# zju3dv/neuralbody

Measured on AMD Instinct MI355X. Metric: ray_samples_per_sec, higher is better.
Workload: dtype f16+f6/f4

## Files before the change

### neuralbody_amd/csrc/nb_march_fold.hip

```cpp
#include "nb_f6_ops.h"
#include "nb_march_hooks.h"

using namespace nbm;

namespace {

#ifndef NB_FP4_TERMS
#define NB_FP4_TERMS 3
#endif
constexpr bool FP4_K[2] = {(NB_FP4_TERMS & 1) != 0, (NB_FP4_TERMS & 2) != 0};
constexpr bool ANY_FP4 = FP4_K[0] || FP4_K[1];
constexpr int TERM_ORDER[2] = {(FP4_K[0] && !FP4_K[1]) ? 1 : 0, (FP4_K[0] && !FP4_K[1]) ? 0 : 1};
__host__ __device__ constexpr int term_pieces(int k) { return FP4_K[k] ? 1 : 2; }
__host__ __device__ constexpr int block_pieces(int mt) { return (4 * mt + mt * term_pieces(0) + mt * term_pieces(1) + 1) & ~1; }
__host__ __device__ constexpr int cross_piece(int mt, int slot, int m) {
    return 4 * mt + (slot == 0 ? 0 : mt * term_pieces(TERM_ORDER[0])) + m * term_pieces(TERM_ORDER[slot]);
}
constexpr int S_R = 8;
__host__ __device__ constexpr int phase_pieces(int nb, int mt) { return nb * block_pieces(mt); }
constexpr int N_PH = 4;
constexpr int PH_NB[N_PH] = {4, 4, 4, 2};
constexpr int PH_MT[N_PH] = {2, 2, 1, 1};
__host__ __device__ constexpr int phase_p0(int ph) {
    int p = 0;
// ... 411 lines not shown
            int worst = 0;
#pragma unroll
            for (int w = 0; w < NW; ++w)
                worst = max(worst, __builtin_amdgcn_readlane(n16[w], 0) + __builtin_amdgcn_readlane(n16[w], 16) +
                                       __builtin_amdgcn_readlane(n16[w], 32) + __builtin_amdgcn_readlane(n16[w], 48));
            p.tier = worst <= K_CAP ? 1 : 2;
        }
    }
    return p;
}

struct TblLoad {
    int rid[2], idx[2];
};
__device__ __forceinline__ TblLoad tbl_issue(const Prep &p, const Lvl &lv, int wave, int os) {
    TblLoad t;
    const float rcp_xy = __builtin_amdgcn_rcpf((float)max(p.nxy, 1)), rcp_x = __builtin_amdgcn_rcpf((float)max(p.nx, 1));
#pragma unroll
    for (int q = 0; q < 2; ++q) {
        const int j = 64 * q + 16 * wave + os;
        t.rid[q] = -1;
        t.idx[q] = -1;
        if (j < p.n) {
            const int vz = (int)(((float)j + 0.5f) * rcp_xy);
            const int r = mad24(vz, -p.nxy, j);
            const int vy = (int)(((float)r + 0.5f) * rcp_x);
            const int vx = mad24(vy, -p.nx, r);
            const int lin = mad24(mad24(p.zlo + vz, lv.H, p.ylo + vy), lv.W, p.xlo + vx);
            t.rid[q] = lv.grid[lin];
            t.idx[q] = p.k0 + j;
        }
    }
    return t;
}
__device__ __forceinline__ void tbl_store(char *actz, const TblLoad &t, const Lvl &lv, unsigned zero_off, int K, int tid) {
    unsigned *tbl = reinterpret_cast<unsigned *>(actz + TBL_OFF);
#pragma unroll
    for (int q = 0; q < 2; ++q)
        if (t.idx[q] >= 0) tbl[t.idx[q]] = t.rid[q] < 0 ? zero_off : (unsigned)(lv.rbase + t.rid[q]) << 10;
    if (tid < 16 && K + tid < ((K + 15) & ~15)) tbl[K + tid] = zero_off;
}
__device__ __forceinline__ void tbl_pass(char *actz, unsigned zero_off, int k_lo, int K, int tid) {
    if (tid >= K_CAP) return;
    unsigned *tbl = reinterpret_cast<unsigned *>(actz + TBL_OFF);
    const int k = k_lo + tid;
    unsigned e = zero_off;
    if (k < K) {
        const int k1 = *reinterpret_cast<const int *>(actz + LVL_OFF + 1 * 32 + 20), k2 = *reinterpret_cast<const int *>(actz + LVL_OFF + 2 * 32 + 20),
                  k3 = *reinterpret_cast<const int *>(actz + LVL_OFF + 3 * 32 + 20);
        const int L = (k >= k1) + (k >= k2) + (k >= k3);
        const i32x4 *lp = reinterpret_cast<const i32x4 *>(actz + LVL_OFF + L * 32);
        const i32x4 b0 = lp[0], b1 = lp[1];
        const Lvl lv = load_lvl(actz, L);
        const int j = k - b1.y;
        const float rcp_xy = __builtin_amdgcn_rcpf((float)max(b1.x, 1)), rcp_x = __builtin_amdgcn_rcpf((float)max(b0.w, 1));
        const int vz = (int)(((float)j + 0.5f) * rcp_xy);
        const int r = mad24(vz, -b1.x, j);
        const int vy = (int)(((float)r + 0.5f) * rcp_x);
        const int vx = mad24(vy, -b0.w, r);
        const int lin = mad24(mad24(b0.z + vz, lv.H, b0.y + vy), lv.W, b0.x + vx);
        const int rid = lv.grid[lin];
        if (rid >= 0) e = (unsigned)(lv.rbase + rid) << 10;
    }
    tbl[tid] = e;
}
__device__ __forceinline__ void lvl_store(char *actz, const Prep &p, int tid, int os, int part) {
    if (tid < 64 && os == 0) {
        i32x4 *d = reinterpret_cast<i32x4 *>(actz + LVL_OFF + part * 32);
        d[0] = i32x4{p.xlo, p.ylo, p.zlo, p.nx};
        d[1] = i32x4{p.nxy, p.k0, p.n, 0};
    }
    if (tid == 0) *reinterpret_cast<int *>(actz + HDR_OFF) = p.K;
}

__device__ __forceinline__ unsigned live_chunks(const char *actz, int lane, int nch, unsigned zero_off) {
    typedef unsigned u32x2 __attribute__((ext_vector_type(2)));
    const u32x2 e = reinterpret_cast<const u32x2 *>(actz + TBL_OFF)[lane];
    const unsigned long long b = __builtin_amdgcn_ballot_w64(lane < 8 * nch && (e.x != zero_off || e.y != zero_off));
    auto half = [](unsigned x) -> unsigned {
        x |= x >> 4;
        x |= x >> 2;
        x |= x >> 1;
        return ((x & 0x01010101u) * 0x00204081u >> 21) & 0xfu;
    };
    return half((unsigned)b) | half((unsigned)(b >> 32)) << 4;
}
__device__ __forceinline__ int pop_chunk(unsigned &m) {
    const int c = __builtin_ctz(m);
    m &= m - 1u;
    return c;
}

struct UCfg {
    int nch, R;
    unsigned live;
    int n_live;
    unsigned ring;
    int ring_off;
};
__device__ __forceinline__ UCfg ucfg_k(int K, unsigned live, unsigned lds_base, int wave) {
    UCfg u;
    u.nch = (K + 15) >> 4;
    const int r = u.nch <= 3 ? u.nch : (u.nch == 4 ? 3 : 2);
    u.live = live;
    u.n_live = __builtin_popcount(live);
    u.R = min(r, u.n_live);
    u.ring_off = WT_CHUNK * u.nch + wave * r * U_CHUNK;
    u.ring = lds_base + (unsigned)u.ring_off;
    return u;
}
__device__ __forceinline__ int list_len(const char *actz) {
    return __builtin_amdgcn_readfirstlane(*reinterpret_cast<const int *>(actz + HDR_OFF));
}
__device__ __forceinline__ void dma_chunk(const MarchArgs &a, const char *actz, int lane, int wave, int c, unsigned dst) {
    const int v = ((lane >> 4) << 2) | ((lane >> 1) & 3);
    const unsigned e = *reinterpret_cast<const unsigned *>(actz + TBL_OFF + (16 * c + v) * 4);
    const unsigned voff0 = e + (unsigned)(64 * wave + 16 * ((lane >> 3) & 1) + 8 * (lane & 1)) * 2u;
    const char *base = a.fold.urows;
#pragma unroll
    for (int form = 0; form < 2; ++form)
#pragma unroll
        for (int m = 0; m < 2; ++m) {
            const unsigned voff = voff0 + form * 512 + m * 64;
            const unsigned d = dst + form * 2048 + m * 1024;
            asm volatile(
                "s_mov_b32 m0, %2\n\t"
                "s_nop 0\n\t"
                "global_load_lds_dwordx4 %0, %1"
                :
                : "v"(voff), "s"(base), "s"(d)
                : "memory", "m0");
        }
}
__device__ __forceinline__ void dma_initial(const MarchArgs &a, const char *actz, int lane, int wave, const UCfg &u) {
    unsigned rest = u.live;
    for (int c = 0; c < u.R; ++c) dma_chunk(a, actz, lane, wave, pop_chunk(rest), u.ring + c * U_CHUNK);
}
__device__ __forceinline__ void dma_wait() { asm volatile("s_waitcnt vmcnt(0)" ::: "memory"); }

__device__ __forceinline__ void wt_build(char *actz, const Lvl &lv, const GridCoord &g, bool take, int wave, int os, int part, int nch,
                                         int k_lo = 0) {
    const int nt = wave >> 1, n = 16 * (wave & 1) + os;
    {
        char *z = actz + (part >> 1) * 2048 + nt * 1024 + ((part & 1) * 32 + n) * 16;
        for (int c = 0; c < nch; ++c) *reinterpret_cast<i32x4 *>(z + c * WT_CHUNK) = i32x4{0, 0, 0, 0};
    }
    if (take) {
        const i32x4 *lp = reinterpret_cast<const i32x4 *>(actz + LVL_OFF + part * 32);
        const i32x4 b0 = lp[0], b1 = lp[1];
        const LvlIdx q = level_index(lv, g);
        const float fx = (float)q.x0, fy = (float)q.y0, fz = (float)q.z0;
        const float wx[2] = {(fx + 1.f) - q.ix, q.ix - fx};
        const float wy[2] = {(fy + 1.f) - q.iy, q.iy - fy};
        const float wz[2] = {(fz + 1.f) - q.iz, q.iz - fz};
        const int kbase = b1.y - k_lo + mad24(q.z0 - b0.z, b1.x, mad24(q.y0 - b0.y, b0.w, q.x0 - b0.x));
        const int sbase = nt * 1024 + n * 16;
        float cw[8];
        int ad[8];
#pragma unroll
        for (int corner = 0; corner < 8; ++corner) {
            const int dx = corner & 1, dy = (corner >> 1) & 1, dz = corner >> 2;
            const int xx = q.x0 + dx, yy = q.y0 + dy, zz = q.z0 + dz;
            const bool inb = (unsigned)xx < (unsigned)lv.W && (unsigned)yy < (unsigned)lv.H && (unsigned)zz < (unsigned)lv.D;
            cw[corner] = (wx[dx] * wy[dy]) * wz[dz];
            const int k = kbase + dx + dy * b0.w + dz * b1.x;
            const int off = ((k << 8) & ~0xfff) | ((k << 6) & 0x200) | ((k << 1) & 0xe);
            ad[corner] = (inb && (unsigned)k < (unsigned)(16 * nch)) ? off + sbase : DUMMY_OFF;
        }
#pragma unroll
        for (int cp = 0; cp < 4; ++cp) {
            const unsigned h = cvt_pk_f16(cw[2 * cp], cw[2 * cp + 1]);
            const unsigned l = cvt_pk_f16(rem16<0>(cw[2 * cp], h), rem16<1>(cw[2 * cp + 1], h));
            *reinterpret_cast<unsigned short *>(actz + ad[2 * cp]) = (unsigned short)(h & 0xffffu);
            *reinterpret_cast<unsigned short *>(actz + ad[2 * cp + 1]) = (unsigned short)(h >> 16);
            *reinterpret_cast<unsigned short *>(actz + ad[2 * cp] + 2048) = (unsigned short)(l & 0xffffu);
            *reinterpret_cast<unsigned short *>(actz + ad[2 * cp + 1] + 2048) = (unsigned short)(l >> 16);
        }
    }
}

__device__ __forceinline__ f16x8 tr_frag(const char *p) {
    const s4v a = __builtin_amdgcn_ds_read_tr16_b64_v4i16((lds_s4p)(p));
    const s4v b = __builtin_amdgcn_ds_read_tr16_b64_v4i16((lds_s4p)(p + 256));
    typedef short s8v __attribute__((ext_vector_type(8)));
    return __builtin_bit_cast(f16x8, s8v{a[0], a[1], a[2], a[3], b[0], b[1], b[2], b[3]});
}
struct FoldFrags {
    f16x8 ah[2], al[2];
    i32x4 bh[2], bl[2];
};
__device__ __forceinline__ void fold_wait(int younger) {
    if (younger >= 2) asm volatile("s_waitcnt vmcnt(8)" ::: "memory");
    else if (younger == 1) asm volatile("s_waitcnt vmcnt(4)" ::: "memory");
    else asm volatile("s_waitcnt vmcnt(0)" ::: "memory");
}
__device__ __forceinline__ void fold_read(FoldFrags &f, const char *ub, const char *wtc) {
#pragma unroll
    for (int m = 0; m < 2; ++m) {
        f.ah[m] = tr_frag(ub + m * 1024);
        f.al[m] = tr_frag(ub + 2048 + m * 1024);
    }
#pragma unroll
    for (int n = 0; n < 2; ++n) {
        f.bh[n] = *reinterpret_cast<const i32x4 *>(wtc + n * 1024);
        f.bl[n] = *reinterpret_cast<const i32x4 *>(wtc + 2048 + n * 1024);
    }
}
__device__ __forceinline__ void fold_mma(const FoldFrags &f, f32x16 (&acc)[2][2]) {
#pragma unroll
    for (int p = 0; p < 3; ++p)
#pragma unroll
        for (int m = 0; m < 2; ++m)
#pragma unroll
            for (int n = 0; n < 2; ++n)
                acc[m][n] = __builtin_amdgcn_mfma_f32_32x32x16_f16(p == 2 ? f.al[m] : f.ah[m], __builtin_bit_cast(f16x8, p == 1 ? f.bl[n] : f.bh[n]),
                                                                   acc[m][n], 0, 0, 0);
}
__device__ __forceinline__ void fold_mfma(const MarchArgs &a, char *actz, int lane, int wave, const UCfg &u, f32x16 (&acc)[2][2],
                                          unsigned *tbuf = nullptr) {
    if (u.n_live == 0) return;
    FOLD_SUB(17);
    const int l15 = lane & 15, g4 = lane >> 4;
    const int tro = (g4 >> 1) * 512 + (g4 & 1) * 128 + (l15 >> 2) * 32 + (l15 & 3) * 8;
    const char *wt = actz + lane * 16;
    const char *ring = actz + u.ring_off + tro;
    int issued = u.R - 1;
    unsigned to_read = u.live, to_fetch = u.live;
    for (int c = 0; c < u.R; ++c) to_fetch &= to_fetch - 1u;
    FoldFrags f0, f1;
    fold_wait(issued);
    FOLD_SUB(18);
    fold_read(f0, ring, wt + pop_chunk(to_read) * WT_CHUNK);
    NB_HOOK_FOLD_FIRST_READ(f0);
    FOLD_SUB(19);
    auto step = [&](FoldFrags &cur, FoldFrags &nxt, int c, int slot) {
        if (c + u.R < u.n_live) {
            asm volatile("s_waitcnt lgkmcnt(0)" : "+v"(cur.ah[0]), "+v"(cur.ah[1]), "+v"(cur.al[0]), "+v"(cur.al[1])::"memory");
            dma_chunk(a, actz, lane, wave, pop_chunk(to_fetch), u.ring + slot * U_CHUNK);
            issued = c + u.R;
        }
        if (c + 1 < u.n_live) {
            const int ns = slot + 1 == u.R ? 0 : slot + 1;
            fold_wait(issued - (c + 1));
            fold_read(nxt, ring + ns * U_CHUNK, wt + pop_chunk(to_read) * WT_CHUNK);
        }
        fold_mma(cur, acc);
    };
    int slot = 0;
    for (int c = 0; c < u.n_live; c += 2) {
        step(f0, f1, c, slot);
        slot = slot + 1 == u.R ? 0 : slot + 1;
        if (c + 1 < u.n_live) {
            step(f1, f0, c + 1, slot);
            slot = slot + 1 == u.R ? 0 : slot + 1;
        }
    }
#pragma unroll
    for (int m = 0; m < 2; ++m) asm volatile("" : "+v"(acc[m][0]), "+v"(acc[m][1]));
    FOLD_SUB(20);
    if (tbuf && lane == 0) tbuf[21] = (unsigned)u.n_live;
}

struct WeightStore4 {
    float q[4] = {0.f, 0.f, 0.f, 0.f};
    __device__ __forceinline__ void push(const MarchArgs &a, long long ray, int s, int S, int part, bool valid, float w) {
        if ((S & 15) != 0) {
            if (valid && part == 0) a.weights[ray * S + s] = w;
            return;
        }
        const int slot = s & 15;
#pragma unroll
        for (int i = 0; i < 4; ++i)
            if (slot == part * 4 + i) q[i] = w;
        if (slot == 15 && valid)
            *reinterpret_cast<f32x4 *>(a.weights + ray * S + (s - 15) + part * 4) = f32x4{q[0], q[1], q[2], q[3]};
    }
};

__device__ __forceinline__ float head_sum(const char *actz, int off, float bias) {
    const f32x4 p = *reinterpret_cast<const f32x4 *>(actz + off);
    return ((p.x + p.y) + (p.z + p.w)) + bias;
}
__device__ __noinline__ void list_ill_ray(const char *actz, const float *pk, float *ill, int cap, int sample, int part, float z_step, int ray) {
    const float *recf = reinterpret_cast<const float *>(actz + RAY_OFF) + sample * RAY_FLOATS;
    const f32x4 c0 = *reinterpret_cast<const f32x4 *>(recf + 12);
    const float sigma_raw = head_sum(actz, SCR_A + sample * 16, pk[P_AB]);
    const bool hit = ray >= 0 && fabsf(sigma_raw) < NB_ILL_SIGMA && c0.x > NB_ILL_T_MIN;
    if (__builtin_amdgcn_ballot_w64(hit) == 0ull) return;
    int slot = -1;
    if (hit && part == 0) slot = atomicAdd(reinterpret_cast<int *>(ill), 1);
    slot = __builtin_amdgcn_ds_bpermute((sample & 15) << 2, slot);
    if (!hit || slot >= cap) return;
    float *irec = ill + NB_ILL_HEADER_FLOATS + (long long)slot * NB_ILL_RECORD_FLOATS;
    if (part == 0) {
        *reinterpret_cast<f32x4 *>(irec) = f32x4{__int_as_float(ray), c0.x, recf[16], recf[17]};
        *reinterpret_cast<f32x4 *>(irec + 4) = f32x4{z_step, __fmul_rn(1e10f, recf[11]), sigma_raw, 0.f};
    } else {
        const int ch = part - 1;
        irec[8 + ch] = part == 1 ? c0.y : (part == 2 ? c0.z : c0.w);
        irec[12 + ch] = head_sum(actz, SCR_C + (ch * 64 + sample) * 16, pk[P_RB + ch]);
    }
}

__device__ __forceinline__ void composite_step(char *actz, const float *pk, int sample, int part, float z_step, float z_after, bool last,
                                               const MarchArgs &a, long long ray, int sidx, int S, bool valid, WeightStore4 &wstore, bool ins) {
    float *recf = reinterpret_cast<float *>(actz + RAY_OFF) + sample * RAY_FLOATS;
    const f32x4 c0 = *reinterpret_cast<const f32x4 *>(recf + 12);
    const float sigma_raw = ins ? head_sum(actz, SCR_A + sample * 16, pk[P_AB]) : 0.f;
    const float d = last ? 1e10f : __fsub_rn(z_after, z_step);
    const float dist = __fmul_rn(d, recf[11]);
    const float sig = fmaxf(sigma_raw, 0.f);
    const float alpha = 1.f - expf(-sig * dist);
    const float w = alpha * c0.x;
    if (part == 0) {
        const float depth = recf[16], accw = recf[17];
        recf[12] = c0.x * (__fadd_rn(__fsub_rn(1.f, alpha), 1e-10f));
        recf[16] = fmaf(w, z_step, depth);
        recf[17] = accw + w;
    } else {
        const int ch = part - 1;
        const float o = ins ? head_sum(actz, SCR_C + (ch * 64 + sample) * 16, pk[P_RB + ch]) : 0.f;
        const float col = part == 1 ? c0.y : (part == 2 ? c0.z : c0.w);
        recf[12 + part] = fmaf(w, 1.f / (1.f + expf(-o)), col);
    }
    wstore.push(a, ray, sidx, S, part, valid, w);
    if (NB_HOOK_RAW_IS_OUTPUT && a.raw && valid && part == 0) {
        float o3[3];
#pragma unroll
        for (int ch = 0; ch < 3; ++ch) o3[ch] = ins ? head_sum(actz, SCR_C + (ch * 64 + sample) * 16, pk[P_RB + ch]) : 0.f;
        *reinterpret_cast<f32x4 *>(a.raw + (ray * S + sidx) * 4) = f32x4{o3[0], o3[1], o3[2], sigma_raw};
    }
}

__host__ __device__ inline int pe_slot_col(int a, int slot) {
    if (a >= 3 || slot >= 30) return -1;
    if (slot == 0) return 256 + 27 + a;
    if (slot <= 20) {
        const int k = (slot - 1) >> 1, is_cos = (slot - 1) & 1;
        return 256 + 27 + 3 + 6 * k + 3 * is_cos + a;
    }
    if (slot == 21) return 256 + a;
    const int k = (slot - 22) >> 1, is_cos = (slot - 22) & 1;
    return 256 + 3 + 6 * k + 3 * is_cos + a;
}

template <int MODE, bool CULL>
__global__ __launch_bounds__(256, 2) void nb_march_fold_kernel(MarchArgs a, const char *stream) {
    constexpr bool POINTS = MODE != 0, DENSITY_ONLY = MODE == 2;
    static_assert(!(CULL && POINTS), "sample culling is a property of the ray march");
    saturate_fp16_conversions();
    __shared__ __attribute__((aligned(16))) char lds[LDS_BYTES];
    char *act = lds;
    const int tid = threadIdx.x;
    const int lane = threadIdx.x & 63, wave = __builtin_amdgcn_readfirstlane(threadIdx.x >> 6);
    const int grp = xcd_remap(blockIdx.x, a.n_wave_groups);
    long long ray = (long long)grp * 64 + 16 * wave + (lane & 15);
    const long long n_units = POINTS ? a.n_pts : a.n_rays;
    bool valid = ray < n_units;
    if (!valid) ray = n_units - 1;
    if (!POINTS && a.ray_order) {
        if (a.ray_order[(long long)grp * 64] == NB_SLOT_DEAD) return;
        const int v = a.ray_order[(long long)grp * 64 + 16 * wave + (lane & 15)];
        valid = v >= 0;
        ray = valid ? v : -(long long)v - 1;
    }
    const int S = POINTS ? 1 : a.n_samples;
    {
        float ox, oy, oz, dx, dy, dz, near, far, dn, vx, vy, vz;
        if constexpr (POINTS) {
            ox = a.wpts[ray * 3 + 0], oy = a.wpts[ray * 3 + 1], oz = a.wpts[ray * 3 + 2];
            dx = DENSITY_ONLY ? 0.f : a.viewdir[ray * 3 + 0], dy = DENSITY_ONLY ? 0.f : a.viewdir[ray * 3 + 1];
            dz = DENSITY_ONLY ? 1.f : a.viewdir[ray * 3 + 2];
            near = far = 0.f;
            dn = 1.f;
            vx = dx, vy = dy, vz = dz;
        } else {
            ox = a.ray_o[ray * 3 + 0], oy = a.ray_o[ray * 3 + 1], oz = a.ray_o[ray * 3 + 2];
            dx = a.ray_d[ray * 3 + 0], dy = a.ray_d[ray * 3 + 1], dz = a.ray_d[ray * 3 + 2];
            near = a.near[ray], far = a.far[ray];
            dn = sqrtf(__fadd_rn(__fadd_rn(__fmul_rn(dx, dx), __fmul_rn(dy, dy)), __fmul_rn(dz, dz)));
            vx = dx / dn, vy = dy / dn, vz = dz / dn;
        }
        if ((lane >> 4) == 0) {
            f32x4 *rec = reinterpret_cast<f32x4 *>(lds + RAY_OFF) + (16 * wave + (lane & 15)) * (RAY_FLOATS / 4);
            rec[0] = f32x4{ox, oy, oz, near};
            rec[1] = f32x4{dx, dy, dz, far};
            rec[2] = f32x4{vx, vy, vz, dn};
            rec[3] = f32x4{1.f, 0.f, 0.f, 0.f};
            rec[4] = f32x4{0.f, 0.f, 0.f, 0.f};
        }
    }
    const float *tr = (!POINTS && a.t_rand) ? a.t_rand + ray * S : nullptr;
    auto tval = [&](int s) -> float { return ((cfloat_ptr)a.t_vals)[s]; };
    auto z_at = [&](int s, float near, float far) -> float {
        if constexpr (POINTS) return 0.f;
        const float zc = z_lin(near, far, tval(s));
        if (!tr) return zc;
        const float lower = s == 0 ? zc : 0.5f * __fadd_rn(zc, z_lin(near, far, tval(s - 1)));
        const float upper = s == S - 1 ? zc : 0.5f * __fadd_rn(z_lin(near, far, tval(s + 1)), zc);
        return __fadd_rn(lower, __fmul_rn(__fsub_rn(upper, lower), tr[s]));
    };

    {
        float *prm = reinterpret_cast<float *>(lds + PRM_OFF);
        for (int i = tid; i < P_SIZE; i += 256) {
            float v;
            if (i < P_B1) v = a.pk[F_OFF_B0 + i - P_B0];
            else if (i < P_B2) v = a.pk[F_OFF_B1 + i - P_B1];
            else if (i < P_AW) v = a.pk[F_OFF_B2 + i - P_B2];
            else if (i < P_RW) v = a.pk[F_OFF_AW + i - P_AW];
            else if (i < P_AB) v = a.pk[F_OFF_RW + i - P_RW];
            else if (i < P_RB) v = a.pk[F_OFF_AB + i - P_AB];
            else if (i < P_LB) v = a.pk[F_OFF_RB + i - P_RB];
            else v = DENSITY_ONLY ? 0.f : a.lb[256 + i - P_LB];
            prm[i] = v;
        }
        if (tid < 4) {
            int *lc = reinterpret_cast<int *>(lds + LC_OFF + tid * 48);
            const unsigned long long gp = (unsigned long long)a.fold.grid[tid];
            lc[0] = a.sc.dhw[tid][0]; lc[1] = a.sc.dhw[tid][1]; lc[2] = a.sc.dhw[tid][2];
            lc[3] = __float_as_int(a.sc.fm1[tid][2]); lc[4] = __float_as_int(a.sc.fm1[tid][1]); lc[5] = __float_as_int(a.sc.fm1[tid][0]);
            lc[6] = __float_as_int(a.sc.fp1[tid][2]); lc[7] = __float_as_int(a.sc.fp1[tid][1]); lc[8] = __float_as_int(a.sc.fp1[tid][0]);
            lc[9] = (int)(unsigned)(gp & 0xffffffffull); lc[10] = (int)(unsigned)(gp >> 32);
            lc[11] = a.fold.row_base[tid];
        }
        __syncthreads();
    }
    const __amdgpu_buffer_rsrc_t wrsrc =
        __builtin_amdgcn_make_buffer_rsrc(const_cast<char *>(stream) + (size_t)wave * WAVE_STREAM, 0, WAVE_STREAM, 0x00020000);
    WRing ring;
    WeightStore4 wstore;
    typedef void __attribute__((address_space(3))) *lptr_t;
    const unsigned lds_base = (unsigned)(unsigned long long)(lptr_t)(lds);

    float z_cur;
    GridCoord g;
    bool ins = true;
    int tier, active;
    auto prep_sequential = [&](int sn, float &z_out, int lane_c) {
        const int os = lane_c & 15, part = lane_c >> 4, sample = 16 * wave + os;
        const f32x4 *rec = reinterpret_cast<const f32x4 *>(lds + RAY_OFF) + sample * (RAY_FLOATS / 4);
        const f32x4 ro = rec[0], rd = rec[1];
        z_out = z_at(sn, ro.w, rd.w);
        const float px = __fadd_rn(ro.x, __fmul_rn(rd.x, z_out)), py = __fadd_rn(ro.y, __fmul_rn(rd.y, z_out)),
                    pz = __fadd_rn(ro.z, __fmul_rn(rd.z, z_out));
        g = grid_coords(a.sc, px, py, pz);
        if constexpr (CULL) ins = cull_inside(a.cull, a.sc, px, py, pz);
        const Lvl lv = load_lvl(lds, part);
        prep_boxes(lds, lv, g, ins, wave, true, os, part);
        __syncthreads();
        const Prep pr = prep_wg<4>(lds, part);
        tier = __builtin_amdgcn_readfirstlane(pr.tier);
        active = __builtin_amdgcn_readfirstlane(pr.any);
        if (tier == 0) {
            const TblLoad tl = tbl_issue(pr, lv, wave, os);
            tbl_store(lds, tl, lv, a.fold.zero_off, pr.K, tid);
        }
        lvl_store(lds, pr, tid, os, part);
    };
    auto fetch_and_weights = [&](int lane_c) {
        if (tier == 0 && active) {
            const int os = lane_c & 15, part = lane_c >> 4;
            const int K = list_len(lds);
            const UCfg u = ucfg_k(K, live_chunks(lds, lane_c, (K + 15) >> 4, a.fold.zero_off), lds_base, wave);
            dma_initial(a, lds, lane_c, wave, u);
            const Lvl lv = load_lvl(lds, part);
            wt_build(lds, lv, g, ins, wave, os, part, u.nch);
        }
    };
    prep_sequential(0, z_cur, lane);
    __syncthreads();
    fetch_and_weights(lane);
    for (int s = 0; s < S; ++s) {
        int zero = 0, lane_i = lane;
        asm volatile("" : "+s"(zero), "+v"(lane_i));
        const int hi = lane_i >> 5, os = lane_i & 15, part = lane_i >> 4, sample = 16 * wave + os;
        const WSrc wl = {wrsrc, (unsigned)lane_i * 16u};
        char *actz = act + zero;
        const float *pk = reinterpret_cast<const float *>(actz + PRM_OFF);
        const f32x4 *rec = reinterpret_cast<const f32x4 *>(actz + RAY_OFF) + sample * (RAY_FLOATS / 4);
        const int sn = sample >> 5, ss = sample & 31;
        const bool more = s + 1 < S;
        const bool ins_cur = ins;
        float z_next = 0.f;
        int tier_next = 0, active_next = 1;
        NB_HOOK_STEP_BEGIN;
        FOLD_STAMP(0);
        __syncthreads();
        FOLD_STAMP(1);
        if (!CULL || active) {
            f32x16 acc[2][2];
            init_bias<2>(pk + P_B0, 2 * wave, hi, acc);
            if (tier == 0) {
                const int K = list_len(actz);
                const UCfg u = ucfg_k(K, live_chunks(actz, lane_i, (K + 15) >> 4, a.fold.zero_off), lds_base, wave);
                fold_mfma(a, actz, lane_i, wave, u, acc, NB_HOOK_TBUF);
            } else if (tier == 3) {
                const Lvl lv = load_lvl(actz, part);
                const int K = list_len(actz);
                for (int k_lo = 0; k_lo < K; k_lo += K_CAP) {
                    tbl_pass(actz, a.fold.zero_off, k_lo, K, tid);
                    __syncthreads();
                    const int kp = min(K - k_lo, K_CAP);
                    const UCfg u = ucfg_k(kp, live_chunks(actz, lane_i, (kp + 15) >> 4, a.fold.zero_off), lds_base, wave);
                    dma_initial(a, actz, lane_i, wave, u);
                    wt_build(actz, lv, g, ins_cur, wave, os, part, u.nch, k_lo);
                    __syncthreads();
                    fold_mfma(a, actz, lane_i, wave, u, acc);
                    __syncthreads();
                }
            } else {
                const Lvl lv = load_lvl(actz, part);
                const int n_groups = tier == 1 ? 4 : 64;
                for (int gi = 0; gi < n_groups; ++gi) {
                    const bool take = ins_cur && (tier == 1 ? wave == gi : sample == gi);
                    prep_boxes(actz, lv, g, take, 0, wave == (tier == 1 ? gi : gi >> 4), os, part);
                    __syncthreads();
                    const Prep pr = prep_wg<1>(actz, part);
                    const TblLoad tl = tbl_issue(pr, lv, wave, os);
                    tbl_store(actz, tl, lv, a.fold.zero_off, pr.K, tid);
                    lvl_store(actz, pr, tid, os, part);
                    __syncthreads();
                    const int kg = list_len(actz);
                    const UCfg u = ucfg_k(kg, live_chunks(actz, lane_i, (kg + 15) >> 4, a.fold.zero_off), lds_base, wave);
                    dma_initial(a, actz, lane_i, wave, u);
                    wt_build(actz, lv, g, take, wave, os, part, u.nch);
                    __syncthreads();
                    fold_mfma(a, actz, lane_i, wave, u, acc);
                    __syncthreads();
                }
            }
            FOLD_DUMP(0, 2)
            FOLD_STAMP(2);
            ring_prime<P_L1>(wl, ring);
            publish_s(actz, lane_i, wave, acc);
            FOLD_STAMP(3);
            init_bias<2>(pk + P_B1, 2 * wave, hi, acc);
            Conv6 pec;
            {
                const f32x4 ro = rec[0], rd = rec[1], rv = rec[2];
                const float xa = part == 0 ? __fadd_rn(ro.x, __fmul_rn(rd.x, z_cur))
                                           : (part == 1 ? __fadd_rn(ro.y, __fmul_rn(rd.y, z_cur)) : __fadd_rn(ro.z, __fmul_rn(rd.z, z_cur)));
                const float va = part == 0 ? rv.x : (part == 1 ? rv.y : rv.z);
                Rev2 tx, tv;
                float e[32];
                auto pe_fill = [&](auto tc) {
                    constexpr int t = decltype(tc)::value;
                    if constexpr (t == 0) {
                        tx = rev2(xa);
                        tv = rev2(va);
                        e[0] = xa;
                        e[21] = va;
                        e[30] = 0.f;
                        e[31] = 0.f;
                    } else if constexpr (t <= 10) {
                        sincos_rev2<t - 1>(tx, e[2 * t - 1], e[2 * t]);
                    } else if constexpr (t <= 14) {
                        sincos_rev2<t - 11>(tv, e[2 * t], e[2 * t + 1]);
                    } else if constexpr (t >= 16) {
                        constexpr int i = t - 16;
                        conv6_pair<2 * i>(pec, e[4 * i], e[4 * i + 1]);
                        conv6_pair<2 * i + 1>(pec, e[4 * i + 2], e[4 * i + 3]);
                    }
                };
                if constexpr (DENSITY_ONLY) layer_s<P_L1, 2, 4, true>(wl, actz, lane_i, ring, acc);
                else layer_s<P_L1, 2, 4, true>(wl, actz, lane_i, ring, acc, pe_fill);
            }
            HalfBlock peh;
            if constexpr (!DENSITY_ONLY) peh = conv6_finish(pec);
            FOLD_DUMP(1, 2)
            FOLD_STAMP(4);
            publish_s(actz, lane_i, wave, acc);
            FOLD_STAMP(5);
            init_bias<2>(pk + P_B2, 2 * wave, hi, acc);
            layer_s<P_L2, 2, 4, true>(wl, actz, lane_i, ring, acc);
            FOLD_DUMP(2, 2)
            FOLD_STAMP(6);
            if (more) {
                const f32x4 ro = rec[0], rd = rec[1];
                z_next = z_at(s + 1, ro.w, rd.w);
                const float px = __fadd_rn(ro.x, __fmul_rn(rd.x, z_next)), py = __fadd_rn(ro.y, __fmul_rn(rd.y, z_next)),
                            pz = __fadd_rn(ro.z, __fmul_rn(rd.z, z_next));
                g = grid_coords(a.sc, px, py, pz);
                if constexpr (CULL) ins = cull_inside(a.cull, a.sc, px, py, pz);
                const Lvl lv = load_lvl(actz, part);
                prep_boxes(actz, lv, g, ins, wave, true, os, part);
            }
            FOLD_STAMP(7);
            if constexpr (DENSITY_ONLY) {
#pragma unroll
                for (int m = 0; m < 2; ++m)
#pragma unroll
                    for (int n = 0; n < 2; ++n)
#pragma unroll
                        for (int r = 0; r < 16; ++r) acc[m][n][r] = relu1(acc[m][n][r]);
            } else {
                publish_s(actz, lane_i, wave, acc);
            }
            FOLD_STAMP(8);
            {
#pragma unroll
                for (int n = 0; n < 2; ++n) {
                    float s4[4] = {0.f, 0.f, 0.f, 0.f};
#pragma unroll
                    for (int m = 0; m < 2; ++m) {
                        const f32x4 *aw = reinterpret_cast<const f32x4 *>(pk + P_AW + hi * 128 + 16 * (2 * wave + m));
#pragma unroll
                        for (int q4 = 0; q4 < 4; ++q4) {
                            const f32x4 w4 = aw[q4];
                            s4[0] = fmaf(w4.x, acc[m][n][4 * q4 + 0], s4[0]);
                            s4[1] = fmaf(w4.y, acc[m][n][4 * q4 + 1], s4[1]);
                            s4[2] = fmaf(w4.z, acc[m][n][4 * q4 + 2], s4[2]);
                            s4[3] = fmaf(w4.w, acc[m][n][4 * q4 + 3], s4[3]);
                        }
                    }
                    float sa = add_halves((s4[0] + s4[1]) + (s4[2] + s4[3]));
                    if (hi == 0) reinterpret_cast<float *>(actz + SCR_A)[(n * 32 + (lane_i & 31)) * 4 + wave] = sa;
                }
            }
            if constexpr (!DENSITY_ONLY) {
                TblLoad tl;
                int k_next = 0;
                if (more) {
                    const Lvl lv = load_lvl(actz, part);
                    const Prep pr = prep_wg<4>(actz, part);
                    tier_next = __builtin_amdgcn_readfirstlane(pr.tier);
                    active_next = __builtin_amdgcn_readfirstlane(pr.any);
                    k_next = __builtin_amdgcn_readfirstlane(pr.K);
                    tl.rid[0] = tl.rid[1] = tl.idx[0] = tl.idx[1] = -1;
                    if (tier_next == 0) tl = tbl_issue(pr, lv, wave, os);
                    lvl_store(actz, pr, tid, os, part);
                }
                FOLD_STAMP(9);
                init_bias<1>(pk + P_LB, wave, hi, acc);
                layer_s<P_VG, 1, 4, false>(wl, actz, lane_i, ring, acc);
                FOLD_STAMP(10);
                if (more && tier_next == 0) {
                    const Lvl lv = load_lvl(actz, part);
                    tbl_store(actz, tl, lv, a.fold.zero_off, k_next, tid);
                }
                __syncthreads();
                ring_prime<P_VP>(wl, ring);
                store_halfblock(actz, part >> 1, part & 1, sn, ss, peh);
                __syncthreads();
                FOLD_STAMP(11);
                layer_s<P_VP, 1, 2, false>(wl, actz, lane_i, ring, acc);
                FOLD_STAMP(12);
                FOLD_DUMP(3, 1)
                {
#pragma unroll
                    for (int n = 0; n < 2; ++n) {
                        float rl[16];
#pragma unroll
                        for (int r = 0; r < 16; ++r) rl[r] = relu1(acc[0][n][r]);
#pragma unroll
                        for (int ch = 0; ch < 3; ++ch) {
                            const f32x4 *rw = reinterpret_cast<const f32x4 *>(pk + P_RW + (ch * 2 + hi) * 64 + 16 * wave);
                            float c4[4] = {0.f, 0.f, 0.f, 0.f};
#pragma unroll
                            for (int q4 = 0; q4 < 4; ++q4) {
                                const f32x4 w4 = rw[q4];
                                c4[0] = fmaf(w4.x, rl[4 * q4 + 0], c4[0]);
                                c4[1] = fmaf(w4.y, rl[4 * q4 + 1], c4[1]);
                                c4[2] = fmaf(w4.z, rl[4 * q4 + 2], c4[2]);
                                c4[3] = fmaf(w4.w, rl[4 * q4 + 3], c4[3]);
                            }
                            float sc = add_halves((c4[0] + c4[1]) + (c4[2] + c4[3]));
                            if (hi == 0) reinterpret_cast<float *>(actz + SCR_C)[(ch * 64 + n * 32 + (lane_i & 31)) * 4 + wave] = sc;
                        }
                    }
                }
            }
        } else if (more) {
            prep_sequential(s + 1, z_next, lane_i);
            tier_next = tier;
            active_next = active;
        }
        FOLD_STAMP(13);
        __syncthreads();
        FOLD_STAMP(14);
        if (more) {
            tier = tier_next;
            active = active_next;
            fetch_and_weights(lane_i);
        }
        FOLD_STAMP(15);
        {
            if constexpr (POINTS) {
                if (valid && part == 0) {
                    const float sigma = head_sum(actz, SCR_A + sample * 16, pk[P_AB]);
                    if constexpr (DENSITY_ONLY) {
                        a.raw_out[ray] = sigma;
                    } else {
                        float o3[3];
#pragma unroll
                        for (int ch = 0; ch < 3; ++ch) o3[ch] = head_sum(actz, SCR_C + (ch * 64 + sample) * 16, pk[P_RB + ch]);
                        *reinterpret_cast<f32x4 *>(a.raw_out + ray * 4) = f32x4{o3[0], o3[1], o3[2], sigma};
                    }
                }
            } else {
                if (s + 1 >= S && a.ill != nullptr)
                    list_ill_ray(actz, pk, a.ill, a.ill_cap, sample, part, z_cur, (valid && (!CULL || ins_cur)) ? (int)ray : -1);
                composite_step(actz, pk, sample, part, z_cur, z_next, s + 1 >= S, a, ray, s, S, valid, wstore, !CULL || ins_cur);
            }
        }
        FOLD_STAMP(16);
        z_cur = z_next;
    }
    if (!POINTS && valid && (lane >> 4) == 0) {
        const f32x4 *rec = reinterpret_cast<const f32x4 *>(lds + RAY_OFF) + (16 * wave + (lane & 15)) * (RAY_FLOATS / 4);
        const f32x4 c0 = rec[3], c1 = rec[4];
        RayAccum ra;
        ra.T = c0.x; ra.cr = c0.y; ra.cg = c0.z; ra.cb = c0.w; ra.depth = c1.x; ra.accw = c1.y;
        ra.store(a, ray);
    }
}

__device__ __forceinline__ int frag_bias_index(int f) {
    const int t = f >> 5, i = f & 31;
    return (t * 2 + ((i >> 2) & 1)) * 16 + (i & 3) + 4 * (i >> 3);
}
__device__ __forceinline__ double frag_row_dot(const float *wfrag, const float *h, int row) {
    const f32x4 *w4 = reinterpret_cast<const f32x4 *>(wfrag) + (size_t)(row >> 5) * 32 * 64 + (row & 31);
    double s = 0.0;
    for (int g = 0; g < 32; ++g)
#pragma unroll
        for (int hi = 0; hi < 2; ++hi) {
            const f32x4 w = w4[g * 64 + hi * 32];
            const float *hh = h + 8 * g + 4 * hi;
            s = fma((double)w.x, (double)hh[0], s);
            s = fma((double)w.y, (double)hh[1], s);
            s = fma((double)w.z, (double)hh[2], s);
            s = fma((double)w.w, (double)hh[3], s);
        }
    return s;
}
__global__ __launch_bounds__(256) void nb_march_fixup_kernel(MarchArgs a) {
    __shared__ float rec[NB_ILL_RECORD_FLOATS];
    __shared__ float cw[32];
    __shared__ int crow[32];
    __shared__ float h[2][256];
    __shared__ double red[4];
    const int tid = threadIdx.x;
    int *hdr = reinterpret_cast<int *>(a.ill);
    const int n = min(hdr[0], a.ill_cap);
    const int S = a.n_samples;
    for (int it = blockIdx.x; it < n; it += gridDim.x) {
        __syncthreads();
        if (tid < NB_ILL_RECORD_FLOATS) rec[tid] = a.ill[NB_ILL_HEADER_FLOATS + (long long)it * NB_ILL_RECORD_FLOATS + tid];
        __syncthreads();
        const long long ray = __float_as_int(rec[0]);
        const float z = rec[4];
        if (tid < 32) {
            const int L = tid >> 3, corner = tid & 7;
            const float px = __fadd_rn(a.ray_o[ray * 3 + 0], __fmul_rn(a.ray_d[ray * 3 + 0], z)),
                        py = __fadd_rn(a.ray_o[ray * 3 + 1], __fmul_rn(a.ray_d[ray * 3 + 1], z)),
                        pz = __fadd_rn(a.ray_o[ray * 3 + 2], __fmul_rn(a.ray_d[ray * 3 + 2], z));
            const GridCoord g = grid_coords(a.sc, px, py, pz);
            Lvl lv;
            lv.D = a.sc.dhw[L][0]; lv.H = a.sc.dhw[L][1]; lv.W = a.sc.dhw[L][2];
            lv.fmx = a.sc.fm1[L][2]; lv.fmy = a.sc.fm1[L][1]; lv.fmz = a.sc.fm1[L][0];
            lv.fpx = a.sc.fp1[L][2]; lv.fpy = a.sc.fp1[L][1]; lv.fpz = a.sc.fp1[L][0];
            const LvlIdx q = level_index(lv, g);
            const float fx = (float)q.x0, fy = (float)q.y0, fz = (float)q.z0;
            const int dx = corner & 1, dy = (corner >> 1) & 1, dz = corner >> 2;
            const float wx = dx ? q.ix - fx : (fx + 1.f) - q.ix, wy = dy ? q.iy - fy : (fy + 1.f) - q.iy, wz = dz ? q.iz - fz : (fz + 1.f) - q.iz;
            const int xx = q.x0 + dx, yy = q.y0 + dy, zz = q.z0 + dz;
            const bool inb = (unsigned)xx < (unsigned)lv.W && (unsigned)yy < (unsigned)lv.H && (unsigned)zz < (unsigned)lv.D;
            int row = -1;
            if (inb) {
                const int rid = a.fold.grid[L][((size_t)zz * lv.H + yy) * lv.W + xx];
                if (rid >= 0) row = a.fold.row_base[L] + rid;
            }
            cw[tid] = (wx * wy) * wz;
            crow[tid] = row;
        }
        __syncthreads();
        {
            double s = (double)a.pk[F_OFF_B0 + frag_bias_index(tid)];
            for (int c = 0; c < 32; ++c) {
                if (crow[c] < 0) continue;
                const _Float16 *u = reinterpret_cast<const _Float16 *>(a.fold.urows) + (size_t)crow[c] * 512;
                s = fma((double)cw[c], (double)(float)u[tid] + (double)(float)u[256 + tid], s);
            }
            h[0][tid] = fmaxf((float)s, 0.f);
        }
        __syncthreads();
        h[1][tid] = fmaxf((float)((double)a.pk[F_OFF_B1 + frag_bias_index(tid)] + frag_row_dot(a.pk + F_OFF_B0 + 256, h[0], tid)), 0.f);
        __syncthreads();
        const float h3 = fmaxf((float)((double)a.pk[F_OFF_B2 + frag_bias_index(tid)] + frag_row_dot(a.pk + F_OFF_B1 + 256, h[1], tid)), 0.f);
        {
            const int t = tid >> 5, i = tid & 31;
            double p = (double)a.pk[F_OFF_AW + ((i >> 2) & 1) * 128 + 16 * t + (i & 3) + 4 * (i >> 3)] * (double)h3;
#pragma unroll
            for (int m = 32; m >= 1; m >>= 1) p += __shfl_xor(p, m);
            if ((tid & 63) == 0) red[tid >> 6] = p;
        }
        __syncthreads();
        if (tid == 0) {
            const float sigma = (float)(((red[0] + red[1]) + (red[2] + red[3])) + (double)a.pk[F_OFF_AB]);
            RayAccum ra;
            ra.T = rec[1]; ra.depth = rec[2]; ra.accw = rec[3];
            ra.cr = rec[8]; ra.cg = rec[9]; ra.cb = rec[10];
            const float out4[4] = {rec[12], rec[13], rec[14], sigma};
            const float w = ra.add(out4, z, rec[5]);
            ra.store(a, ray);
            a.weights[ray * S + (S - 1)] = w;
            if (a.raw) a.raw[(ray * S + (S - 1)) * 4 + 3] = sigma;
            if ((sigma > 0.f) != (rec[6] > 0.f)) atomicAdd(&hdr[1], 1);
        }
    }
}

__device__ __forceinline__ int phase_col(int ph, int b, int kh, int e) {
    if (ph < 3) return col_hidden(32 * b + e, kh);
    return pe_slot_col(2 * b + kh, e);
}
__device__ __forceinline__ float phase_weight(const nb_mlp_params &p, const float *f32_blob, int ph, int row, int b, int kh, int e) {
    const int col = phase_col(ph, b, kh, e);
    if (col < 0) return 0.f;
    if (ph == 0) return p.fc1_w[row * 256 + col];
    if (ph == 1) return p.fc2_w[row * 256 + col];
    if (ph == 2) {
        const int tt = col >> 5, rr = col & 31, hi2 = (rr >> 2) & 1, r2 = (rr & 3) + 4 * (rr >> 3), q2 = 16 * tt + r2;
        double s = 0.0;
        for (int m = 0; m < 256; ++m)
            s += (double)p.view_w[row * 346 + m] *
                 (double)f32_blob[F_OFF_L4 + (((m >> 5) * 32 + (q2 >> 2)) * 64 + (hi2 * 32 + (m & 31))) * 4 + (q2 & 3)];
        return (float)s;
    }
    return p.view_w[row * 346 + col];
}

__device__ __forceinline__ unsigned fp4_e2m1_bits(float v) {
    const unsigned sgn = v < 0.f ? 8u : 0u;
    const float a = fminf(fabsf(v), 6.f);
    constexpr float grid[8] = {0.f, 0.5f, 1.f, 1.5f, 2.f, 3.f, 4.f, 6.f};
    unsigned code = 0;
    float best = a;
    for (unsigned c = 1; c < 8; ++c) {
        const float d = fabsf(a - grid[c]);
        if (d < best || (d == best && (c & 1u) == 0u)) {
            best = d;
            code = c;
        }
    }
    return sgn | code;
}

__global__ void nb_pack_fold_kernel(nb_mlp_params p, const float *__restrict__ f32_blob, unsigned *__restrict__ out, int *__restrict__ stats) {
    const int t = blockIdx.x * blockDim.x + threadIdx.x;
    if (t >= 4 * P_TOTAL * 64) return;
    const int lane = t & 63, piece = (t >> 6) % P_TOTAL, w = (t >> 6) / P_TOTAL;
    const int i = lane & 31, kg = lane >> 5;
    int ph = 0, p0 = 0;
    for (int q = 0; q < N_PH; ++q) {
        const int n = phase_pieces(PH_NB[q], PH_MT[q]);
        if (piece < p0 + n) {
            ph = q;
            break;
        }
        p0 += n;
    }
    const int mt = PH_MT[ph], ppb = block_pieces(mt);
    const int rel = piece - p0, b = rel / ppb, r = rel % ppb;
    unsigned w32[4] = {0u, 0u, 0u, 0u};
    if (r < 4 * mt) {
        const int j = r / mt, m = r % mt;
        const int row = (mt == 2 ? 64 * w + 32 * m : 32 * w) + i;
        for (int q = 0; q < 8; q += 2) {
            const f16x2 hp = {(_Float16)phase_weight(p, f32_blob, ph, row, b, kg, 8 * j + q),
                              (_Float16)phase_weight(p, f32_blob, ph, row, b, kg, 8 * j + q + 1)};
            w32[q / 2] = __builtin_bit_cast(unsigned, hp);
        }
    } else {
        int r6 = r - 4 * mt, k = -1, m = 0, half = 0;
        for (int slot = 0; slot < 2; ++slot) {
            const int kk = TERM_ORDER[slot], width = mt * term_pieces(kk);
            if (r6 < width) {
                k = kk;
                m = r6 / term_pieces(kk);
                half = r6 % term_pieces(kk);
                break;
            }
            r6 -= width;
        }
        if (k >= 0) {
            const bool four = FP4_K[k];
            const float top = four ? 6.f : 7.5f;
            const int row = (mt == 2 ? 64 * w + 32 * m : 32 * w) + i;
            float wv[32], amax = 0.f;
            for (int e = 0; e < 32; ++e) {
                const int n = k ? e : 16 * (e & 1) + (e >> 1);
                const float wt = phase_weight(p, f32_blob, ph, row, b, kg, n);
                const float h = (float)(_Float16)wt;
                wv[e] = k ? wt - h : h;
                amax = fmaxf(amax, fabsf(wv[e]));
            }
            int ex = 0;
            if (amax > 0.f && amax < 3.0e38f) {
                ex = ilogbf(amax / top);
                if (ldexpf(top, ex) < amax) ++ex;
                ex = min(max(ex, -120), 120);
            }
            if (four) {
                for (int e = 0; e < 32; ++e) w32[e >> 3] |= fp4_e2m1_bits(ldexpf(wv[e], -ex)) << (4 * (e & 7));
                unsigned char *sc = reinterpret_cast<unsigned char *>(out) + (size_t)w * WAVE_STREAM + (size_t)P_TOTAL * 1024 +
                                    (size_t)(phase_s0(ph) + b) * 256 + lane * 4 + (k * mt + m);
                *sc = (unsigned char)(127 + ex);
            } else {
                unsigned w8[8] = {0u, 0u, 0u, 0u, 0u, 0u, 0u, 0u};
                for (int e = 0; e < 32; ++e) {
                    const unsigned code = fp6_e2m3_bits(ldexpf(wv[e], -ex));
                    const int bit = 6 * e;
                    w8[bit >> 5] |= code << (bit & 31);
                    if ((bit & 31) > 26) w8[(bit >> 5) + 1] |= code >> (32 - (bit & 31));
                }
                w8[6] = (unsigned)(127 + ex);
                for (int q = 0; q < 4; ++q) w32[q] = w8[4 * half + q];
            }
            if (k == 0 && half == 0) {
                int small = 0, nz = 0;
                for (int e = 0; e < 32; ++e) {
                    nz += wv[e] != 0.f;
                    small += wv[e] != 0.f && fabsf(wv[e]) < 0.125f * amax;
                }
                const int layer = ph < 2 ? ph : 2;
                atomicAdd(&stats[2 * layer], small);
                atomicAdd(&stats[2 * layer + 1], nz);
            }
        }
    }
    unsigned *dst = reinterpret_cast<unsigned *>(reinterpret_cast<char *>(out) + (size_t)w * WAVE_STREAM) + ((size_t)piece * 64 + lane) * 4;
    for (int q = 0; q < 4; ++q) dst[q] = w32[q];
}

}

namespace nbm {

long long fold_stream_floats() { return (long long)4 * WAVE_STREAM / 4 + 8; }

int pack_fold_stream(const nb_mlp_params *p, float *packed, long long stream_off, hipStream_t st) {
    const long long n = (long long)4 * P_TOTAL * 64;
    int *stats = reinterpret_cast<int *>(packed + stream_off + (long long)4 * WAVE_STREAM / 4);
    NB_REQUIRE(hipMemsetAsync(stats, 0, 8 * sizeof(int), st) == hipSuccess, "pack_fold_stream: hipMemsetAsync failed");
    hipLaunchKernelGGL(nb_pack_fold_kernel, dim3(nb_ceil_div(n, 256)), dim3(256), 0, st, *p, packed,
                       reinterpret_cast<unsigned *>(packed + stream_off), stats);
    NB_CHECK_LAUNCH("nb_pack_fold_kernel");
    return NB_OK;
}

int launch_march_fold(MarchArgs a, long long stream_off, hipStream_t st) {
    a.n_wave_groups = (int)nb_ceil_div(a.ray_order ? a.n_slots : a.n_rays, 64);
    const char *stream = reinterpret_cast<const char *>(a.pk + stream_off);
    if (a.ill) NB_REQUIRE(hipMemsetAsync(a.ill, 0, NB_ILL_HEADER_FLOATS * sizeof(float), st) == hipSuccess, "nb_march: hipMemsetAsync(ill_scratch) failed");
    if (a.cull.n_views) hipLaunchKernelGGL((nb_march_fold_kernel<0, true>), dim3(a.n_wave_groups), dim3(256), 0, st, a, stream);
    else hipLaunchKernelGGL((nb_march_fold_kernel<0, false>), dim3(a.n_wave_groups), dim3(256), 0, st, a, stream);
    NB_CHECK_LAUNCH("nb_march_fold_kernel");
    if (a.ill) {
        hipLaunchKernelGGL(nb_march_fixup_kernel, dim3(NB_ILL_FIXUP_BLOCKS), dim3(256), 0, st, a);
        NB_CHECK_LAUNCH("nb_march_fixup_kernel");
    }
    return NB_OK;
}

int launch_points_fold(MarchArgs a, int density_only, long long stream_off, hipStream_t st) {
    a.n_wave_groups = (int)nb_ceil_div(a.n_pts, 64);
    const char *stream = reinterpret_cast<const char *>(a.pk + stream_off);
    if (density_only) hipLaunchKernelGGL((nb_march_fold_kernel<2, false>), dim3(a.n_wave_groups), dim3(256), 0, st, a, stream);
    else hipLaunchKernelGGL((nb_march_fold_kernel<1, false>), dim3(a.n_wave_groups), dim3(256), 0, st, a, stream);
    NB_CHECK_LAUNCH("nb_march_fold_kernel (points)");
    return NB_OK;
}

}
```

Before: 1.423 billion.

## Defer compositing math and interleave it into the next step's matmul layer

Splits the per-sample compositing into a stage step, which writes pre-activation values to a pending LDS area, and seven slices (exp, sigmoid, accumulate) that run during the next iteration's view-layer matmul through a fill callback. The goal is to hide the transcendental and LDS latency of compositing behind the MLP layer rather than paying for it serially after the sync. Weight pushes are delayed by one sample, and the last sample is flushed explicitly. This adds more LDS traffic and code complexity, and it risks ordering bugs across the deferred state.

After: 1.420 billion. Within noise of the previous version (-0.2%).

```diff
diff --git a/neuralbody_amd/csrc/nb_march_fold.hip b/neuralbody_amd/csrc/nb_march_fold.hip
--- a/neuralbody_amd/csrc/nb_march_fold.hip
+++ b/neuralbody_amd/csrc/nb_march_fold.hip
@@ -737,34 +737,70 @@
     }
 }
 
-__device__ __forceinline__ void composite_step(char *actz, const float *pk, int sample, int part, float z_step, float z_after, bool last,
-                                               const MarchArgs &a, long long ray, int sidx, int S, bool valid, WeightStore4 &wstore, bool ins) {
+
+constexpr int PEND_OFF = SCR_C + 1024;
+constexpr int COMPOSITE_SLICES = 7;
+struct Pending {
+    float x, T, acc;
+    float e;
+    float f, c, w;
+};
+__device__ __forceinline__ void composite_stage(char *actz, const float *pk, int sample, int part, float z_step, float z_after, bool last,
+                                                const MarchArgs &a, long long ray, int sidx, int S, bool valid, bool ins) {
     float *recf = reinterpret_cast<float *>(actz + RAY_OFF) + sample * RAY_FLOATS;
-    const f32x4 c0 = *reinterpret_cast<const f32x4 *>(recf + 12);
     const float sigma_raw = ins ? head_sum(actz, SCR_A + sample * 16, pk[P_AB]) : 0.f;
+    const int ch = max(part - 1, 0);
+    const float o = ins ? head_sum(actz, SCR_C + (ch * 64 + sample) * 16, pk[P_RB + ch]) : 0.f;
+    if (NB_HOOK_RAW_IS_OUTPUT && a.raw && valid && part == 0) {
+        float o3[3];
+#pragma unroll
+        for (int c = 0; c < 3; ++c) o3[c] = ins ? head_sum(actz, SCR_C + (c * 64 + sample) * 16, pk[P_RB + c]) : 0.f;
+        *reinterpret_cast<f32x4 *>(a.raw + (ray * S + sidx) * 4) = f32x4{o3[0], o3[1], o3[2], sigma_raw};
+    }
     const float d = last ? 1e10f : __fsub_rn(z_after, z_step);
     const float dist = __fmul_rn(d, recf[11]);
     const float sig = fmaxf(sigma_raw, 0.f);
-    const float alpha = 1.f - expf(-sig * dist);
-    const float w = alpha * c0.x;
-    if (part == 0) {
-        const float depth = recf[16], accw = recf[17];
-        recf[12] = c0.x * (__fadd_rn(__fsub_rn(1.f, alpha), 1e-10f));
-        recf[16] = fmaf(w, z_step, depth);
-        recf[17] = accw + w;
+    reinterpret_cast<float *>(actz + PEND_OFF + sample * 16)[part] = part == 0 ? __fmul_rn(-sig, dist) : o;
+    if (part == 0) recf[18] = z_step;
+}
+template <int I>
+__device__ __forceinline__ void composite_slice(Pending &p, char *actz, int sample, int part) {
+#pragma clang fp contract(off)
+    float *recf = reinterpret_cast<float *>(actz + RAY_OFF) + sample * RAY_FLOATS;
+    const float *pend = reinterpret_cast<const float *>(actz + PEND_OFF + sample * 16);
+    if constexpr (I == 0) {
+        p.x = pend[0];
+        p.T = recf[12];
+        p.acc = recf[17];
+    } else if constexpr (I == 1) {
+        p.e = expf(p.x);
+    } else if constexpr (I == 2) {
+        const float alpha = 1.f - p.e;
+        const float w = alpha * p.T;
+        recf[12] = p.T * ((1.f - alpha) + 1e-10f);
+        recf[17] = p.acc + w;
+        recf[19] = w;
+    } else if constexpr (I == 3) {
+        p.e = pend[max(part, 1)];
+    } else if constexpr (I == 4) {
+        p.e = expf(-p.e);
+    } else if constexpr (I == 5) {
+        p.e = 1.f / (1.f + p.e);
+        p.f = recf[18];
+        p.c = recf[part == 0 ? 16 : 12 + part];
+        p.w = recf[19];
     } else {
-        const int ch = part - 1;
-        const float o = ins ? head_sum(actz, SCR_C + (ch * 64 + sample) * 16, pk[P_RB + ch]) : 0.f;
-        const float col = part == 1 ? c0.y : (part == 2 ? c0.z : c0.w);
-        recf[12 + part] = fmaf(w, 1.f / (1.f + expf(-o)), col);
-    }
-    wstore.push(a, ray, sidx, S, part, valid, w);
-    if (NB_HOOK_RAW_IS_OUTPUT && a.raw && valid && part == 0) {
-        float o3[3];
-#pragma unroll
-        for (int ch = 0; ch < 3; ++ch) o3[ch] = ins ? head_sum(actz, SCR_C + (ch * 64 + sample) * 16, pk[P_RB + ch]) : 0.f;
-        *reinterpret_cast<f32x4 *>(a.raw + (ray * S + sidx) * 4) = f32x4{o3[0], o3[1], o3[2], sigma_raw};
-    }
+        static_assert(I == COMPOSITE_SLICES - 1, "slices");
+        recf[part == 0 ? 16 : 12 + part] = fmaf(p.w, part == 0 ? p.f : p.e, p.c);
+    }
+}
+__device__ __forceinline__ void composite_flush(char *actz, int sample, int part) {
+    Pending p;
+    sfor<0, COMPOSITE_SLICES>([&](auto ic) { composite_slice<decltype(ic)::value>(p, actz, sample, part); });
+}
+__device__ __forceinline__ void composite_push(const char *actz, int sample, int part, const MarchArgs &a, long long ray, int sidx, int S,
+                                               bool valid, WeightStore4 &wstore) {
+    wstore.push(a, ray, sidx, S, part, valid, (reinterpret_cast<const float *>(actz + RAY_OFF) + sample * RAY_FLOATS)[19]);
 }
 
 __host__ __device__ inline int pe_slot_col(int a, int slot) {
@@ -823,6 +859,7 @@
             rec[2] = f32x4{vx, vy, vz, dn};
             rec[3] = f32x4{1.f, 0.f, 0.f, 0.f};
             rec[4] = f32x4{0.f, 0.f, 0.f, 0.f};
+            if constexpr (!POINTS) *reinterpret_cast<f32x4 *>(lds + PEND_OFF + (16 * wave + (lane & 15)) * 16) = f32x4{-0.f, 0.f, 0.f, 0.f};
         }
     }
     const float *tr = (!POINTS && a.t_rand) ? a.t_rand + ray * S : nullptr;
@@ -1068,7 +1105,17 @@
                 }
                 FOLD_STAMP(9);
                 init_bias<1>(pk + P_LB, wave, hi, acc);
-                layer_s<P_VG, 1, 4, false>(wl, actz, lane_i, ring, acc);
+                if constexpr (POINTS) {
+                    layer_s<P_VG, 1, 4, false>(wl, actz, lane_i, ring, acc);
+                } else {
+                    Pending pend;
+                    auto comp_fill = [&](auto tc) {
+                        constexpr int t = decltype(tc)::value;
+                        if constexpr (t % 3 == 1 && t / 3 < COMPOSITE_SLICES)
+                            composite_slice<t / 3>(pend, actz, sample, part);
+                    };
+                    layer_s<P_VG, 1, 4, false>(wl, actz, lane_i, ring, acc, comp_fill);
+                }
                 FOLD_STAMP(10);
                 if (more && tier_next == 0) {
                     const Lvl lv = load_lvl(actz, part);
@@ -1106,10 +1153,13 @@
                     }
                 }
             }
-        } else if (more) {
-            prep_sequential(s + 1, z_next, lane_i);
-            tier_next = tier;
-            active_next = active;
+        } else {
+            composite_flush(actz, sample, part);
+            if (more) {
+                prep_sequential(s + 1, z_next, lane_i);
+                tier_next = tier;
+                active_next = active;
+            }
         }
         FOLD_STAMP(13);
         __syncthreads();
@@ -1136,7 +1186,12 @@
             } else {
                 if (s + 1 >= S && a.ill != nullptr)
                     list_ill_ray(actz, pk, a.ill, a.ill_cap, sample, part, z_cur, (valid && (!CULL || ins_cur)) ? (int)ray : -1);
-                composite_step(actz, pk, sample, part, z_cur, z_next, s + 1 >= S, a, ray, s, S, valid, wstore, !CULL || ins_cur);
+                composite_push(actz, sample, part, a, ray, s - 1, S, valid && s > 0, wstore);
+                composite_stage(actz, pk, sample, part, z_cur, z_next, s + 1 >= S, a, ray, s, S, valid, !CULL || ins_cur);
+                if (s + 1 >= S) {
+                    composite_flush(actz, sample, part);
+                    composite_push(actz, sample, part, a, ray, s, S, valid, wstore);
+                }
             }
         }
         FOLD_STAMP(16);
```
